# Orange-OpenSource/AIVC

Hardware: AMD Instinct MI355X
Metric: encode+decode fps @1080p YUV420 (RA GOP32) (higher is better)
Workload: dtype f32; 1 GPU; 1920x1080 8-bit YUV420, coding structure 1_GOP_32: one 128-frame clip = 4 intra-period units of 33 frames (132 coded frames, the last 4 repeat the last frame) encoded + decoded per step; synthetic random-init stand-in for model ms_ssim-4 (widths {'n2': 64, 'n': 128, 'c_y': 64, 'c_short': 64, 'c_z': 32, 'n_h': 128}), last analysis conv calibrated so that 6 (MOFNet) / 12 (CodecNet) of the 64 y featu; parallelism=single GPU

## Files before the change

### aivc_amd/csrc/conv_wino.hip

```cpp
#include <stdlib.h>

#include <type_traits>
#include <utility>

#include "common.h"

namespace aivc {

typedef float floatx16 __attribute__((ext_vector_type(16)));

struct WinoArgs {
  aivc_conv_params p;
  int TH, TW;
  int nby, nbx;
  int gy;
  int total;
  int poly;
  int cpp_shift;
};

__device__ __forceinline__ void wino_glds16(const float *base, uint32_t voff, uint32_t lds_dst) {
  asm volatile("s_mov_b32 m0, %2\n\ts_nop 0\n\tglobal_load_lds_dwordx4 %0, %1" : : "v"(voff), "s"(base), "s"(lds_dst) : "memory", "m0");
}

constexpr int WINO_RAW_STAGE = 11 * 1024;
constexpr int WINO_U_STAGE = 32 * 1024;
constexpr int WINO_V_QUAD = 1152;
constexpr int WINO_V_POS = 2 * WINO_V_QUAD;
constexpr int WINO_V_STAGE = 16 * WINO_V_POS;
constexpr int WINO_LDS = 2 * (WINO_RAW_STAGE + WINO_U_STAGE + WINO_V_STAGE);

__device__ __attribute__((aligned(4096))) float wino_zeros[1024];

template <int MODE>
__global__ __launch_bounds__(512) void conv_wino_kernel(WinoArgs a) {
  constexpr bool POLY = MODE == 1, TC = MODE == 2;
  extern __shared__ __attribute__((aligned(16))) char wsmem[];
  char *raw = wsmem, *Us = wsmem + 2 * WINO_RAW_STAGE, *Vs = Us + 2 * WINO_U_STAGE;
  const uint32_t lds0 = (uint32_t)(uintptr_t)(__attribute__((address_space(3))) char *)wsmem;

  const aivc_conv_params &p = a.p;
  const int tid = threadIdx.x, lane = tid & 63;
  const int wave = __builtin_amdgcn_readfirstlane(tid >> 6);
  const int ph = wave >> 2, wm = (wave >> 1) & 1, wn = wave & 1;
  const int H = TC ? p.h_in : p.h_out, W = TC ? p.w_in : p.w_out, Hi = p.h_in, Wi = p.w_in, Cin = p.c_in, Cout = p.c_out;
  const int gyc = TC ? 4 * a.gy : a.gy;
  constexpr int poly = POLY ? 1 : 0;
  const int cpp_shift = a.cpp_shift, cpp_mask = (1 << a.cpp_shift) - 1;

  const uint32_t total = (uint32_t)a.total, nwg = gridDim.x, xcd = blockIdx.x & 7u, slot = blockIdx.x >> 3;
  const uint32_t per_xcd = (total + 7u) >> 3, wg_per_xcd = (nwg + 7u - xcd) >> 3;
  const uint32_t x_lo = xcd * per_xcd, x_hi = min(x_lo + per_xcd, total);
  auto block_of = [&](uint32_t k) -> uint32_t { return x_lo + slot + k * wg_per_xcd; };
  const uint32_t n_mine = x_lo + slot < x_hi ? (x_hi - x_lo - slot + wg_per_xcd - 1u) / wg_per_xcd : 0u;
  if (n_mine == 0u) return;
  struct Desc {
    const float *xbase, *ubase;
    uint32_t r_off[2];
    int img, byi, bxi, cb;
  };
  int s_quad[2], s_py[2], s_px[2];
#pragma unroll
  for (int k = 0; k < 2; ++k) {
    int sl = 64 * (wave + 8 * k) + lane;
    sl = sl < 648 ? sl : 647;
    const int q2 = sl >> 1, plane = q2 / 81, rem = q2 - plane * 81, hy = rem / 9, hx = rem - hy * 9;
    s_quad[k] = sl & 1;
    s_py[k] = 2 * hy + (plane >> 1);
    s_px[k] = 2 * hx + (plane & 1);
  }
  const int nch = poly ? 4 * (Cin >> 3) : (Cin >> 3);
  auto make_desc = [&](uint32_t blk) {
    Desc d;
    d.cb = (int)(blk % (uint32_t)gyc);
    uint32_t rest = blk / (uint32_t)gyc;
    d.bxi = (int)(rest % (uint32_t)a.nbx);
    rest /= (uint32_t)a.nbx;
    d.byi = (int)(rest % (uint32_t)a.nby);
    d.img = (int)(rest / (uint32_t)a.nby);
    d.xbase = p.x + (size_t)d.img * (size_t)Hi * Wi * Cin;
    d.ubase = p.w_wino + (size_t)d.cb * (size_t)nch * (WINO_U_STAGE / 4);
    if constexpr (MODE == 0) {
#pragma unroll
      for (int k = 0; k < 2; ++k) {
        const int iy = max(min(16 * d.byi - 1 + s_py[k], Hi - 1), 0), ix = max(min(16 * d.bxi - 1 + s_px[k], Wi - 1), 0);
        d.r_off[k] = ((uint32_t)(iy * Wi + ix) * (uint32_t)Cin + (uint32_t)(4 * s_quad[k])) * 4u;
      }
    }
    return d;
  };
  uint32_t iss_off[2];
  auto patch_offsets = [&](const Desc &d_, int ph2) {
    const int st = poly ? 2 : 1, py = ph2 >> 1, px = ph2 & 1;
#pragma unroll
    for (int k = 0; k < 2; ++k) {
      const int iy = max(min(st * (16 * d_.byi - 1 + s_py[k]) + py, Hi - 1), 0), ix = max(min(st * (16 * d_.bxi - 1 + s_px[k]) + px, Wi - 1), 0);
      iss_off[k] = ((uint32_t)(iy * Wi + ix) * (uint32_t)Cin + (uint32_t)(4 * s_quad[k])) * 4u;
    }
  };
  uint64_t iss_addr[2];
  auto tc_addresses = [&](const Desc &d_) {
#pragma unroll
    for (int k = 0; k < 2; ++k) {
      const int iy = 16 * d_.byi - 1 + s_py[k], ix = 16 * d_.bxi - 1 + s_px[k];
      const bool in = iy >= 0 && iy < Hi && ix >= 0 && ix < Wi;
      const uint64_t a_in = (uint64_t)(uintptr_t)d_.xbase + ((uint64_t)((uint32_t)(iy * Wi + ix)) * (uint32_t)Cin + (uint32_t)(4 * s_quad[k])) * 4u;
      const uint64_t a_z = (uint64_t)(uintptr_t)wino_zeros + (uint32_t)(16 * s_quad[k]);
      iss_addr[k] = in ? a_in : a_z;
    }
  };
  Desc cur = make_desc(block_of(0)), nxt = n_mine > 1u ? make_desc(block_of(1)) : cur;

  const uint32_t r_dst = __builtin_amdgcn_readfirstlane(lds0 + (uint32_t)wave * 1024u);
  const uint32_t u_dst = __builtin_amdgcn_readfirstlane(lds0 + (uint32_t)(2 * WINO_RAW_STAGE) + (uint32_t)wave * 4096u);
  const uint32_t u_off = (uint32_t)(wave * 4096 + lane * 16);
  auto uniform_ptr = [](const float *q) -> const float * {
    const uint64_t v = (uint64_t)(uintptr_t)q;
    const uint32_t lo = __builtin_amdgcn_readfirstlane((uint32_t)v), hi = __builtin_amdgcn_readfirstlane((uint32_t)(v >> 32));
    return reinterpret_cast<const float *>((uintptr_t)(((uint64_t)hi << 32) | lo));
  };
  auto issue_raw = [&](const Desc &d_, int c) {
    const uint32_t d = r_dst + (uint32_t)((c & 1) * WINO_RAW_STAGE);
    if constexpr (TC) {
      if (c == 0) tc_addresses(d_);
      const uint32_t du = __builtin_amdgcn_readfirstlane(d);
      asm volatile("s_mov_b32 m0, %1\n\ts_nop 0\n\tglobal_load_lds_dwordx4 %0, off" : : "v"(iss_addr[0]), "s"(du) : "memory", "m0");
      if (wave < 3) asm volatile("s_mov_b32 m0, %1\n\ts_nop 0\n\tglobal_load_lds_dwordx4 %0, off" : : "v"(iss_addr[1]), "s"(du + 8192u) : "memory", "m0");
      iss_addr[0] += 32u;
      iss_addr[1] += 32u;
    } else if constexpr (POLY) {
      if ((c & cpp_mask) == 0) patch_offsets(d_, c >> cpp_shift);
      const float *src = uniform_ptr(d_.xbase + 8 * (c & cpp_mask));
      const uint32_t du = __builtin_amdgcn_readfirstlane(d);
      wino_glds16(src, iss_off[0], du);
      if (wave < 3) wino_glds16(src, iss_off[1], du + 8192u);
    } else {
      const float *src = d_.xbase + 8 * c;
      wino_glds16(src, d_.r_off[0], d);
      if (wave < 3) wino_glds16(src, d_.r_off[1], d + 8192u);
    }
  };
  auto zero_pos = [&](int pc, int i, int j) -> bool {
    if constexpr (POLY) return ((pc >> 1) && i == 3) || ((pc & 1) && j == 3);
    if constexpr (TC) return ((pc >> 1) && i == 0) || ((pc & 1) && j == 0);
    return false;
  };
  auto phase_or_class = [&](const Desc &d_, int c) -> int { return POLY ? c >> cpp_shift : (TC ? d_.cb / a.gy : 0); };
  auto issue_u = [&](const Desc &d_, int c) {
    const float *src = MODE != 0 ? uniform_ptr(d_.ubase + (size_t)c * (WINO_U_STAGE / 4)) : d_.ubase + (size_t)c * (WINO_U_STAGE / 4);
    const uint32_t d = MODE != 0 ? __builtin_amdgcn_readfirstlane(u_dst + (uint32_t)((c & 1) * WINO_U_STAGE)) : u_dst + (uint32_t)((c & 1) * WINO_U_STAGE);
    bool lo = true, hi = true;
    if constexpr (MODE != 0) {
      const int pc = phase_or_class(d_, c), i = wave >> 1, j = 2 * (wave & 1);
      lo = !zero_pos(pc, i, j);
      hi = !zero_pos(pc, i, j + 1);
    }
    if (lo && hi) {
      asm volatile("s_mov_b32 m0, %2\n\ts_nop 0\n\t"
                   "global_load_lds_dwordx4 %0, %1\n\t"
                   "global_load_lds_dwordx4 %0, %1 offset:1024\n\t"
                   "global_load_lds_dwordx4 %0, %1 offset:2048\n\t"
                   "global_load_lds_dwordx4 %0, %1 offset:3072"
                   : : "v"(u_off), "s"(src), "s"(d) : "memory", "m0");
    } else if (lo) {
      asm volatile("s_mov_b32 m0, %2\n\ts_nop 0\n\t"
                   "global_load_lds_dwordx4 %0, %1\n\t"
                   "global_load_lds_dwordx4 %0, %1 offset:1024"
                   : : "v"(u_off), "s"(src), "s"(d) : "memory", "m0");
    } else if (hi) {
      asm volatile("s_mov_b32 m0, %2\n\ts_nop 0\n\t"
                   "global_load_lds_dwordx4 %0, %1 offset:2048\n\t"
                   "global_load_lds_dwordx4 %0, %1 offset:3072"
                   : : "v"(u_off), "s"(src), "s"(d) : "memory", "m0");
    }
  };

  const int l32 = lane & 31;
  const int t_grp = (l32 < 4 || (l32 >= 12 && l32 < 16) || (l32 >= 20 && l32 < 28)) ? 0 : 1;
  const int t_pos = t_grp == 0 ? (l32 < 4 ? l32 : (l32 < 16 ? l32 - 8 : l32 - 12)) : (l32 < 12 ? l32 - 4 : (l32 < 20 ? l32 - 8 : l32 - 16));
  const int t_quad = t_pos >> 3, t_tx = (t_pos & 7) ^ (t_grp << 2), t_ty = ((tid >> 6) & 1) * 4 + (lane >> 5) * 2 + t_grp;
  const int t_i = __builtin_amdgcn_readfirstlane(tid >> 7);
  const int t_ra = t_i == 0 ? 0 : (t_i == 2 ? 2 : 1), t_rb = t_i == 3 ? 3 : (t_i == 2 ? 1 : 2);
  const float t_si = t_i == 1 ? 1.0f : -1.0f;
  const int t_base = ((t_ty * 9 + t_tx) * 2 + t_quad) * 16;
  auto pix_off = [](int r, int c) { return (((r & 1) * 2 + (c & 1)) * 81 + (r >> 1) * 9 + (c >> 1)) * 32; };
  int t_oa[4], t_ob[4];
#pragma unroll
  for (int c = 0; c < 4; ++c) {
    t_oa[c] = t_base + pix_off(t_ra, c);
    t_ob[c] = t_base + pix_off(t_rb, c);
  }
  const int t_vdst = (4 * t_i) * WINO_V_POS + t_quad * WINO_V_QUAD + (t_ty * 8 + t_tx) * 16;
  float4 R[4];
  auto comb = [](const float4 &u, const float4 &v, float sgn) {
    float4 o;
    o.x = __builtin_fmaf(sgn, v.x, u.x);
    o.y = __builtin_fmaf(sgn, v.y, u.y);
    o.z = __builtin_fmaf(sgn, v.z, u.z);
    o.w = __builtin_fmaf(sgn, v.w, u.w);
    return o;
  };
  auto transform_step = [&](auto STAGE, auto STEP) {
    constexpr int st = decltype(STEP)::value, stage = decltype(STAGE)::value;
    const char *rs = raw + stage * WINO_RAW_STAGE;
    char *vd = Vs + stage * WINO_V_STAGE + t_vdst;
    if constexpr (st < 4) {
      const float4 xa = *reinterpret_cast<const float4 *>(rs + t_oa[st]), xb = *reinterpret_cast<const float4 *>(rs + t_ob[st]);
      R[st] = comb(xa, xb, t_si);
    } else if constexpr (st == 4) {
      *reinterpret_cast<float4 *>(vd) = comb(R[0], R[2], -1.0f);
    } else if constexpr (st == 5) {
      *reinterpret_cast<float4 *>(vd + WINO_V_POS) = comb(R[1], R[2], 1.0f);
    } else if constexpr (st == 6) {
      *reinterpret_cast<float4 *>(vd + 2 * WINO_V_POS) = comb(R[2], R[1], -1.0f);
    } else {
      *reinterpret_cast<float4 *>(vd + 3 * WINO_V_POS) = comb(R[1], R[3], -1.0f);
    }
  };
  auto transform0 = [&]() {
    using std::integral_constant;
    using Z = integral_constant<int, 0>;
    transform_step(Z{}, integral_constant<int, 0>{});
    transform_step(Z{}, integral_constant<int, 1>{});
    transform_step(Z{}, integral_constant<int, 2>{});
    transform_step(Z{}, integral_constant<int, 3>{});
    transform_step(Z{}, integral_constant<int, 4>{});
    transform_step(Z{}, integral_constant<int, 5>{});
    transform_step(Z{}, integral_constant<int, 6>{});
    transform_step(Z{}, integral_constant<int, 7>{});
  };

  floatx16 acc[8];
#pragma unroll
  for (int q = 0; q < 8; ++q)
#pragma unroll
    for (int r = 0; r < 16; ++r) acc[q][r] = 0.0f;
  const int hh = lane >> 5, l31 = lane & 31;
  const int a_rd = (8 * ph) * WINO_V_POS + hh * WINO_V_QUAD + (32 * wm + l31) * 16;
  const int b_rd = (8 * ph) * 2048 + hh * 1024 + (32 * wn + l31) * 16;
  auto multiply = [&](auto STAGE, auto FIRST, uint32_t tm, uint32_t pm) {
    constexpr int stage = decltype(STAGE)::value;
    constexpr bool first = decltype(FIRST)::value;
    using NEXT = std::integral_constant<int, 1 - stage>;
    const char *va = Vs + stage * WINO_V_STAGE + a_rd, *ub = Us + stage * WINO_U_STAGE + b_rd;
    float4 af[2][2], bf[2][2];
    auto rd = [&](int set, int q) {
      af[set][0] = *reinterpret_cast<const float4 *>(va + q * WINO_V_POS);
      bf[set][0] = *reinterpret_cast<const float4 *>(ub + q * 2048);
      af[set][1] = *reinterpret_cast<const float4 *>(va + (q + 1) * WINO_V_POS);
      bf[set][1] = *reinterpret_cast<const float4 *>(ub + (q + 1) * 2048);
    };
    rd(0, 0);
    auto pair = [&](auto Q) {
      constexpr int q = decltype(Q)::value, set = (q >> 1) & 1;
      using std::integral_constant;
      if constexpr (q + 2 < 8) {
        if (MODE == 0 || (first && !TC) || (pm & (0xCu << q))) rd(1 - set, q + 2);
      }
      __builtin_amdgcn_sched_barrier(0);
      const float4 x0 = af[set][0], y0 = bf[set][0], x1 = af[set][1], y1 = bf[set][1];
#ifdef WINO_EXP_NOMFMA
      acc[q][0] += x0.x * y0.x + x0.y * y0.y + x0.z * y0.z + x0.w * y0.w;
      acc[q + 1][0] += x1.x * y1.x + x1.y * y1.y + x1.z * y1.z + x1.w * y1.w;
#else
      if constexpr (first && TC) {
        const floatx16 zero = {0.0f, 0.0f, 0.0f, 0.0f, 0.0f, 0.0f, 0.0f, 0.0f, 0.0f, 0.0f, 0.0f, 0.0f, 0.0f, 0.0f, 0.0f, 0.0f};
        if ((pm >> q) & 1u) {
          acc[q] = __builtin_amdgcn_mfma_f32_32x32x2f32(x0.x, y0.x, zero, 0, 0, 0);
          acc[q] = __builtin_amdgcn_mfma_f32_32x32x2f32(x0.y, y0.y, acc[q], 0, 0, 0);
          acc[q] = __builtin_amdgcn_mfma_f32_32x32x2f32(x0.z, y0.z, acc[q], 0, 0, 0);
          acc[q] = __builtin_amdgcn_mfma_f32_32x32x2f32(x0.w, y0.w, acc[q], 0, 0, 0);
        } else {
          acc[q] = __builtin_amdgcn_mfma_f32_32x32x2f32(0.0f, 0.0f, zero, 0, 0, 0);
        }
        if ((pm >> (q + 1)) & 1u) {
          acc[q + 1] = __builtin_amdgcn_mfma_f32_32x32x2f32(x1.x, y1.x, zero, 0, 0, 0);
          acc[q + 1] = __builtin_amdgcn_mfma_f32_32x32x2f32(x1.y, y1.y, acc[q + 1], 0, 0, 0);
          acc[q + 1] = __builtin_amdgcn_mfma_f32_32x32x2f32(x1.z, y1.z, acc[q + 1], 0, 0, 0);
          acc[q + 1] = __builtin_amdgcn_mfma_f32_32x32x2f32(x1.w, y1.w, acc[q + 1], 0, 0, 0);
        } else {
          acc[q + 1] = __builtin_amdgcn_mfma_f32_32x32x2f32(0.0f, 0.0f, zero, 0, 0, 0);
        }
      } else if constexpr (first) {
        const floatx16 zero = {0.0f, 0.0f, 0.0f, 0.0f, 0.0f, 0.0f, 0.0f, 0.0f, 0.0f, 0.0f, 0.0f, 0.0f, 0.0f, 0.0f, 0.0f, 0.0f};
        acc[q] = __builtin_amdgcn_mfma_f32_32x32x2f32(x0.x, y0.x, zero, 0, 0, 0);
        acc[q + 1] = __builtin_amdgcn_mfma_f32_32x32x2f32(x1.x, y1.x, zero, 0, 0, 0);
        acc[q] = __builtin_amdgcn_mfma_f32_32x32x2f32(x0.y, y0.y, acc[q], 0, 0, 0);
        acc[q + 1] = __builtin_amdgcn_mfma_f32_32x32x2f32(x1.y, y1.y, acc[q + 1], 0, 0, 0);
        acc[q] = __builtin_amdgcn_mfma_f32_32x32x2f32(x0.z, y0.z, acc[q], 0, 0, 0);
        acc[q + 1] = __builtin_amdgcn_mfma_f32_32x32x2f32(x1.z, y1.z, acc[q + 1], 0, 0, 0);
        acc[q] = __builtin_amdgcn_mfma_f32_32x32x2f32(x0.w, y0.w, acc[q], 0, 0, 0);
        acc[q + 1] = __builtin_amdgcn_mfma_f32_32x32x2f32(x1.w, y1.w, acc[q + 1], 0, 0, 0);
      } else {
        if (MODE == 0 || ((pm >> q) & 1u)) {
          acc[q] = __builtin_amdgcn_mfma_f32_32x32x2f32(x0.x, y0.x, acc[q], 0, 0, 0);
          acc[q] = __builtin_amdgcn_mfma_f32_32x32x2f32(x0.y, y0.y, acc[q], 0, 0, 0);
          acc[q] = __builtin_amdgcn_mfma_f32_32x32x2f32(x0.z, y0.z, acc[q], 0, 0, 0);
          acc[q] = __builtin_amdgcn_mfma_f32_32x32x2f32(x0.w, y0.w, acc[q], 0, 0, 0);
        }
        if (MODE == 0 || ((pm >> (q + 1)) & 1u)) {
          acc[q + 1] = __builtin_amdgcn_mfma_f32_32x32x2f32(x1.x, y1.x, acc[q + 1], 0, 0, 0);
          acc[q + 1] = __builtin_amdgcn_mfma_f32_32x32x2f32(x1.y, y1.y, acc[q + 1], 0, 0, 0);
          acc[q + 1] = __builtin_amdgcn_mfma_f32_32x32x2f32(x1.z, y1.z, acc[q + 1], 0, 0, 0);
          acc[q + 1] = __builtin_amdgcn_mfma_f32_32x32x2f32(x1.w, y1.w, acc[q + 1], 0, 0, 0);
        }
      }
#endif
      __builtin_amdgcn_sched_barrier(0);
#ifndef WINO_EXP_NOXFORM
      if ((tm >> q) & 1u) transform_step(NEXT{}, integral_constant<int, q>{});
      if ((tm >> (q + 1)) & 1u) transform_step(NEXT{}, integral_constant<int, q + 1>{});
#endif
      __builtin_amdgcn_sched_barrier(0);
    };
    using std::integral_constant;
    pair(integral_constant<int, 0>{});
    pair(integral_constant<int, 2>{});
    pair(integral_constant<int, 4>{});
    pair(integral_constant<int, 6>{});
  };

  auto issue_raw_at = [&](uint32_t kb, int c) {
    if (c < nch) issue_raw(cur, c);
    else if (kb + 1u < n_mine) issue_raw(nxt, c - nch);
  };
  auto issue_u_at = [&](uint32_t kb, int c) {
    if (c < nch) issue_u(cur, c);
    else if (kb + 1u < n_mine) issue_u(nxt, c - nch);
  };
  issue_raw(cur, 0);
  issue_u(cur, 0);
  issue_raw_at(0u, 1);
  asm volatile("s_waitcnt vmcnt(0)" ::: "memory");
  __builtin_amdgcn_s_barrier();
  transform0();
  asm volatile("s_waitcnt lgkmcnt(0)" ::: "memory");
  __builtin_amdgcn_s_barrier();
  const int act1 = p.act1, act2 = p.act2;
  auto act_cheap = [](int act, float v) {
    const float neg = act == AIVC_ACT_LEAKY ? v * 0.01f : (act == AIVC_ACT_RELU ? 0.0f : v);
    return v > 0.0f ? v : neg;
  };
  for (uint32_t kb = 0; kb < n_mine; ++kb) {
    auto chunk = [&](auto STAGE, auto FIRST, int c) {
#ifndef WINO_EXP_NODMA
      issue_raw_at(kb, c + 2);
      issue_u_at(kb, c + 1);
#endif
      uint32_t pm = 0xFFu;
      if (poly) {
        const int ph2 = c >> cpp_shift;
        pm = 0xFFu & ~((ph2 & 1) ? 0x88u : 0u) & ~(((ph2 >> 1) && ph) ? 0xF0u : 0u);
      }
      if constexpr (TC) {
        const int cls = cur.cb / a.gy;
        pm = 0xFFu & ~((cls & 1) ? 0x11u : 0u) & ~(((cls >> 1) && !ph) ? 0x0Fu : 0u);
      }
      uint32_t tm = (c + 1 < nch || kb + 1u < n_mine) ? 0xFFu : 0u;
      if constexpr (MODE != 0) {
        const int pcn = c + 1 < nch ? phase_or_class(cur, c + 1) : phase_or_class(nxt, 0);
        if (zero_pos(pcn, t_i, 1)) tm = 0u;
        else if (zero_pos(pcn, 1, POLY ? 3 : 0)) tm &= POLY ? ~0x80u : ~0x10u;
      }
      multiply(STAGE, FIRST, tm, pm);
      asm volatile("s_waitcnt vmcnt(0) lgkmcnt(0)" ::: "memory");
      __builtin_amdgcn_s_barrier();
    };
    {
      using std::integral_constant;
      using S0 = integral_constant<int, 0>;
      using S1 = integral_constant<int, 1>;
      chunk(S0{}, std::true_type{}, 0);
      chunk(S1{}, std::false_type{}, 1);
      for (int c = 2; c < nch; c += 2) {
        chunk(S0{}, std::false_type{}, c);
        chunk(S1{}, std::false_type{}, c + 1);
      }
    }

#ifdef WINO_EXP_NOEPI
    if (kb + 1u < n_mine) { cur = nxt; if (kb + 2u < n_mine) nxt = make_desc(block_of(kb + 2u)); continue; }
#endif
    floatx16 keep[2], give[2];
    auto fold = [&](auto PH) {
      constexpr int phc = decltype(PH)::value;
#pragma unroll
      for (int bb = 0; bb < 2; ++bb)
#pragma unroll
        for (int r = 0; r < 16; ++r) keep[bb][r] = give[bb][r] = 0.0f;
#pragma unroll
      for (int q = 0; q < 8; ++q) {
        const int i = 2 * phc + (q >> 2), j = q & 3;
        const int t0i = i < 3 ? 1 : 0, t1i = i == 0 ? 0 : (i == 1 ? 1 : -1);
        const int t0j = j < 3 ? 1 : 0, t1j = j == 0 ? 0 : (j == 1 ? 1 : -1);
#pragma unroll
        for (int o = 0; o < 4; ++o) {
          const int cf = ((o >> 1) ? t1i : t0i) * ((o & 1) ? t1j : t0j);
          floatx16 &dst = (o >> 1) == phc ? keep[o & 1] : give[o & 1];
          if (cf > 0) {
#pragma unroll
            for (int r = 0; r < 16; ++r) dst[r] = dst[r] + acc[q][r];
          } else if (cf < 0) {
#pragma unroll
            for (int r = 0; r < 16; ++r) dst[r] = dst[r] - acc[q][r];
          }
        }
      }
    };
    if (ph) fold(std::integral_constant<int, 1>{});
    else fold(std::integral_constant<int, 0>{});
    {
      float *xch = reinterpret_cast<float *>(Vs + WINO_V_STAGE) + wave * 1024;
      const float *theirs = reinterpret_cast<const float *>(Vs + WINO_V_STAGE) + (wave ^ 4) * 1024;
#pragma unroll
      for (int bb = 0; bb < 2; ++bb) {
#pragma unroll
        for (int r = 0; r < 16; ++r) xch[r * 64 + lane] = give[bb][r];
        asm volatile("s_waitcnt lgkmcnt(0)" ::: "memory");
        __builtin_amdgcn_s_barrier();
#pragma unroll
        for (int r = 0; r < 16; ++r) keep[bb][r] = keep[bb][r] + theirs[r * 64 + lane];
        asm volatile("s_waitcnt lgkmcnt(0)" ::: "memory");
        __builtin_amdgcn_s_barrier();
      }
    }

    {
      const float *__restrict__ g_mul = p.mul;
      const float *__restrict__ g_res = p.res;
      float *__restrict__ g_y = p.y;
      const int cls = TC ? cur.cb / a.gy : 0, pyc = cls >> 1, pxc = cls & 1;
      const int OS = TC ? 2 : 1;
      const int Wo_ = OS * W, Ho_ = OS * H;
      const int co = (TC ? cur.cb - cls * a.gy : cur.cb) * 64 + 32 * wn + l31;
      const bool has_bias = p.bias != nullptr;
      const float cbias = has_bias ? p.bias[co] : 0.0f;
      const int oy_w = 2 * (8 * cur.byi + 4 * wm) + ph;
      const bool inside_x = 16 * cur.bxi + 16 <= W;
      if (!g_mul && act1 != AIVC_ACT_SIGMOID) {
        const int cols_left = W - 16 * cur.bxi;
        typedef __attribute__((address_space(1))) char gchar;
        typedef __attribute__((address_space(1))) float gfloat;
        typedef __attribute__((address_space(1))) const float cgfloat;
        const uint32_t c4 = (uint32_t)Cout * 4u, sx = (uint32_t)OS * c4;
        uint32_t lane_b = (uint32_t)(2 * (8 * cur.bxi + 4 * hh)) * sx + (uint32_t)pxc * c4 + (uint32_t)co * 4u;
        asm volatile("" : "+v"(lane_b));
        const size_t img_b = (size_t)cur.img * (size_t)Ho_ * Wo_ * c4;
        auto rows = [&](auto RES, auto KIND, auto EDGE) {
          constexpr bool has_res = decltype(RES)::value;
          constexpr bool edge = decltype(EDGE)::value;
          constexpr int kind = decltype(KIND)::value;
          bool ok[8];
#pragma unroll
          for (int rr = 0; rr < 4; ++rr)
#pragma unroll
            for (int b = 0; b < 2; ++b) ok[rr * 2 + b] = !edge || 2 * (4 * hh + rr) + b < cols_left;
#pragma unroll
          for (int rq = 0; rq < 4; ++rq) {
            const int oy = oy_w + 2 * rq;
            if (oy >= H) continue;
            const size_t row_b = img_b + (size_t)(OS * oy + pyc) * Wo_ * c4;
            gchar *yb = (gchar *)(uintptr_t)(reinterpret_cast<char *>(g_y) + row_b);
            const gchar *rb = (const gchar *)(uintptr_t)(reinterpret_cast<const char *>(g_res) + row_b);
            float rv[8];
            if constexpr (has_res) {
#pragma unroll
              for (int rr = 0; rr < 4; ++rr)
#pragma unroll
                for (int b = 0; b < 2; ++b)
                  rv[rr * 2 + b] = ok[rr * 2 + b] ? *reinterpret_cast<cgfloat *>(rb + lane_b + (uint32_t)((2 * rr + b) * 512) * (sx / 512u)) : 0.0f;
            }
#pragma unroll
            for (int rr = 0; rr < 4; ++rr)
#pragma unroll
              for (int b = 0; b < 2; ++b) {
                const int r = rq * 4 + rr;
                float v = keep[b][r];
                if (has_bias) v = v + cbias;
                if constexpr (kind == 1) v = __builtin_fmaxf(v, v * 0.01f);
                if constexpr (kind == 2) v = v > 0.0f ? v : 0.0f;
                if constexpr (has_res) v = v + rv[rr * 2 + b];
                if constexpr (kind == 3) v = v > 0.0f ? v : 0.0f;
                if constexpr (kind == 4) v = __builtin_fmaxf(v, v * 0.01f);
#ifdef WINO_EXP_NOSTORE
                if (v == 123.456f)
#endif
                if (ok[rr * 2 + b]) *reinterpret_cast<gfloat *>(yb + lane_b + (uint32_t)((2 * rr + b) * 512) * (sx / 512u)) = v;
              }
          }
        };
        using std::integral_constant;
        int kind = -1;
        if (act1 == AIVC_ACT_NONE && act2 == AIVC_ACT_NONE) kind = 0;
        else if (act2 == AIVC_ACT_NONE) kind = act1 == AIVC_ACT_LEAKY ? 1 : 2;
        else if (act1 == AIVC_ACT_NONE) kind = act2 == AIVC_ACT_RELU ? 3 : 4;
        if (kind >= 0 && sx % 512u == 0u) {
          auto go = [&](auto RES, auto EDGE) {
            switch (kind) {
              case 0: rows(RES, integral_constant<int, 0>{}, EDGE); break;
              case 1: rows(RES, integral_constant<int, 1>{}, EDGE); break;
              case 2: rows(RES, integral_constant<int, 2>{}, EDGE); break;
              case 3: rows(RES, integral_constant<int, 3>{}, EDGE); break;
              default: rows(RES, integral_constant<int, 4>{}, EDGE); break;
            }
          };
          if (inside_x) {
            if (g_res) go(integral_constant<bool, true>{}, integral_constant<bool, false>{});
            else go(integral_constant<bool, false>{}, integral_constant<bool, false>{});
          } else {
            if (g_res) go(integral_constant<bool, true>{}, integral_constant<bool, true>{});
            else go(integral_constant<bool, false>{}, integral_constant<bool, true>{});
          }
          goto epilogue_done;
        }
      }
      {
        const size_t ybase = (size_t)cur.img * (size_t)Ho_ * Wo_ * Cout + (size_t)co;
#pragma unroll
        for (int r = 0; r < 16; ++r) {
          const int t = (r & 3) + 8 * (r >> 2) + 4 * hh;
          const int oy = oy_w + 2 * (t >> 3), ox0 = 2 * (8 * cur.bxi + (t & 7));
          if (oy >= H) continue;
#pragma unroll
          for (int b = 0; b < 2; ++b) {
            const int ox = ox0 + b;
            if (ox >= W) continue;
            const size_t o = ybase + ((size_t)(OS * oy + pyc) * Wo_ + (size_t)(OS * ox + pxc)) * (size_t)Cout;
            float v = keep[b][r];
            if (has_bias) v = v + cbias;
            v = act_cheap(act1, v);
            if (g_mul) v = g_mul[o] * v;
            if (g_res) v = v + g_res[o];
            v = act_cheap(act2, v);
#ifdef WINO_EXP_NOSTORE
            if (v == 123.456f)
#endif
            g_y[o] = v;
          }
        }
      }
    epilogue_done:;
    }
    cur = nxt;
    if (kb + 2u < n_mine) nxt = make_desc(block_of(kb + 2u));
  }
}

__device__ __forceinline__ void wino_g(double g0, double g1, double g2, double (&out)[4]) {
  out[0] = g0;
  out[1] = 0.5 * ((g0 + g1) + g2);
  out[2] = 0.5 * ((g0 - g1) + g2);
  out[3] = g2;
}
__global__ void __launch_bounds__(256) winograd_weights_kernel(const float *w, int c_out, int c_in, float *u) {
  const size_t idx = (size_t)blockIdx.x * 256 + threadIdx.x;
  if (idx >= (size_t)c_out * c_in) return;
  const int co = (int)(idx / c_in), ci = (int)(idx % c_in);
  double t[4][3], uu[4][4];
#pragma unroll
  for (int l = 0; l < 3; ++l) {
    double col[4];
    wino_g((double)w[(((size_t)co * 3 + 0) * 3 + l) * c_in + ci], (double)w[(((size_t)co * 3 + 1) * 3 + l) * c_in + ci],
           (double)w[(((size_t)co * 3 + 2) * 3 + l) * c_in + ci], col);
#pragma unroll
    for (int i = 0; i < 4; ++i) t[i][l] = col[i];
  }
#pragma unroll
  for (int i = 0; i < 4; ++i) wino_g(t[i][0], t[i][1], t[i][2], uu[i]);
#pragma unroll
  for (int i = 0; i < 4; ++i)
#pragma unroll
    for (int j = 0; j < 4; ++j) u[AIVC_WINO_U_INDEX(co, 4 * i + j, ci, c_in)] = (float)uu[i][j];
}

int winograd_weights(const float *w, int c_out, int c_in, float *u, hipStream_t s) {
  hipLaunchKernelGGL(winograd_weights_kernel, dim3(cdiv((size_t)c_out * c_in, 256)), dim3(256), 0, s, w, c_out, c_in, u);
  return check_launch("winograd_weights");
}

__global__ void __launch_bounds__(256) winograd_weights_poly5_kernel(const float *w, int c_out, int c_in, float *u) {
  const size_t idx = (size_t)blockIdx.x * 256 + threadIdx.x;
  if (idx >= (size_t)c_out * c_in * 4) return;
  const int phase = (int)(idx % 4), ci = (int)((idx / 4) % c_in), co = (int)(idx / ((size_t)4 * c_in));
  const int py = phase >> 1, px = phase & 1;
  auto tap = [&](int r, int l) -> double {
    const int ky = 2 * r + py, kx = 2 * l + px;
    return ky < 5 && kx < 5 ? (double)w[(((size_t)co * 5 + ky) * 5 + kx) * c_in + ci] : 0.0;
  };
  double t[4][3], uu[4][4];
#pragma unroll
  for (int l = 0; l < 3; ++l) {
    double col[4];
    wino_g(tap(0, l), tap(1, l), tap(2, l), col);
#pragma unroll
    for (int i = 0; i < 4; ++i) t[i][l] = col[i];
  }
#pragma unroll
  for (int i = 0; i < 4; ++i) wino_g(t[i][0], t[i][1], t[i][2], uu[i]);
#pragma unroll
  for (int i = 0; i < 4; ++i)
#pragma unroll
    for (int j = 0; j < 4; ++j) u[AIVC_WINO_U_INDEX(co, 4 * i + j, phase * c_in + ci, 4 * c_in)] = (float)uu[i][j];
}

int winograd_weights_poly5(const float *w, int c_out, int c_in, float *u, hipStream_t s) {
  hipLaunchKernelGGL(winograd_weights_poly5_kernel, dim3(cdiv((size_t)c_out * c_in * 4, 256)), dim3(256), 0, s, w, c_out, c_in, u);
  return check_launch("winograd_weights_poly5");
}

__global__ void __launch_bounds__(256) winograd_weights_tconv5_kernel(const float *w, int c_out, int c_in, float *u) {
  const size_t idx = (size_t)blockIdx.x * 256 + threadIdx.x;
  if (idx >= (size_t)c_out * c_in * 4) return;
  const int ci = (int)(idx % c_in), co = (int)((idx / c_in) % c_out), cls = (int)(idx / ((size_t)c_in * c_out));
  const int pyc = cls >> 1, pxc = cls & 1;
  auto tap = [&](int r, int l) -> double {
    const int ky = pyc + 4 - 2 * r, kx = pxc + 4 - 2 * l;
    return ky < 5 && kx < 5 ? (double)w[(((size_t)co * 5 + ky) * 5 + kx) * c_in + ci] : 0.0;
  };
  double t[4][3], uu[4][4];
#pragma unroll
  for (int l = 0; l < 3; ++l) {
    double col[4];
    wino_g(tap(0, l), tap(1, l), tap(2, l), col);
#pragma unroll
    for (int i = 0; i < 4; ++i) t[i][l] = col[i];
  }
#pragma unroll
  for (int i = 0; i < 4; ++i) wino_g(t[i][0], t[i][1], t[i][2], uu[i]);
#pragma unroll
  for (int i = 0; i < 4; ++i)
#pragma unroll
    for (int j = 0; j < 4; ++j) u[AIVC_WINO_U_INDEX(cls * c_out + co, 4 * i + j, ci, c_in)] = (float)uu[i][j];
}

int winograd_weights_tconv5(const float *w, int c_out, int c_in, float *u, hipStream_t s) {
  hipLaunchKernelGGL(winograd_weights_tconv5_kernel, dim3(cdiv((size_t)c_out * c_in * 4, 256)), dim3(256), 0, s, w, c_out, c_in, u);
  return check_launch("winograd_weights_tconv5");
}

bool conv2d_wino_supported(const aivc_conv_params &p) {
  if (!aivc_winograd_covers(&p) || p.gdn) return false;
  if ((uint64_t)p.h_in * p.w_in * p.c_in * 4u >= 0xFFFF0000ull) return false;
  const bool tc = p.mode == AIVC_MODE_TCONV;
  if (tc && p.c_in > 960) return false;
  const uint64_t gh = tc ? p.h_in : p.h_out, gw = tc ? p.w_in : p.w_out;
  const uint64_t blocks = (uint64_t)p.n * ((gh + 15) / 16) * ((gw + 15) / 16) * ((uint64_t)p.c_out / 64) * (tc ? 4 : 1);
  return blocks < 0x7FFFFFFFull;
}

int conv2d_wino_variant(const aivc_conv_params &p) { return p.mode == AIVC_MODE_TCONV ? 303 : (p.ksize == 5 ? 302 : 301); }

template <int MODE>
static int wino_launch(const WinoArgs &a, unsigned grid, hipStream_t s) {
  static LdsOptIn opt_in;
  if (!opt_in.raise(reinterpret_cast<const void *>(conv_wino_kernel<MODE>), WINO_LDS)) return check_launch("conv_wino lds attribute");
  hipLaunchKernelGGL(conv_wino_kernel<MODE>, dim3(grid), dim3(512), WINO_LDS, s, a);
  return check_launch("conv_wino");
}

int conv2d_wino(const aivc_conv_params &p, hipStream_t s) {
  if (!conv2d_wino_supported(p) || !p.w_wino) return AIVC_ERR_UNSUPPORTED;
  const bool tc = p.mode == AIVC_MODE_TCONV;
  WinoArgs a;
  a.p = p;
  a.poly = !tc && p.ksize == 5 ? 1 : 0;
  a.cpp_shift = 0;
  while ((8 << a.cpp_shift) < p.c_in) ++a.cpp_shift;
  a.TH = ((tc ? p.h_in : p.h_out) + 1) / 2;
  a.TW = ((tc ? p.w_in : p.w_out) + 1) / 2;
  a.nby = (a.TH + 7) / 8;
  a.nbx = (a.TW + 7) / 8;
  a.gy = p.c_out / 64;
  a.total = (int)((size_t)p.n * a.nby * a.nbx * a.gy * (tc ? 4 : 1));
  static std::atomic<int> n_cu{0};
  if (n_cu.load(std::memory_order_relaxed) == 0) {
    int dev = 0, cus = 0;
    n_cu = hipGetDevice(&dev) == hipSuccess && hipDeviceGetAttribute(&cus, hipDeviceAttributeMultiprocessorCount, dev) == hipSuccess && cus > 0 ? cus : 256;
  }
  unsigned grid = (unsigned)n_cu.load(std::memory_order_relaxed);
  if ((unsigned)a.total < grid) grid = (unsigned)a.total;
  if (tc) return wino_launch<2>(a, grid, s);
  return a.poly ? wino_launch<1>(a, grid, s) : wino_launch<0>(a, grid, s);
}

}
```

Baseline: 95.63 frames/s.

## Defer last MFMA pair of each Winograd chunk past next chunk's DMA issue

Moves the q=6 MFMA pair of each chunk into the start of the following chunk, where it runs after that chunk's raw/U global-to-LDS DMAs are issued. The aim is to issue the loads earlier and overlap the outstanding MFMAs with them, shortening the stall at the end-of-chunk waitcnt and barrier. The fragment registers are hoisted to kernel scope, so the previous chunk's operands stay live across the barrier; this raises register pressure and relies on the deferred pair still reading valid registers. The change also adds an optional LDS cycle-stamp probe, built only under WINO_STAMPS.

```diff
diff --git a/aivc_amd/csrc/conv_wino.hip b/aivc_amd/csrc/conv_wino.hip
--- a/aivc_amd/csrc/conv_wino.hip
+++ b/aivc_amd/csrc/conv_wino.hip
@@ -4,6 +4,10 @@
 #include <utility>
 
 #include "common.h"
+
+#ifndef WINO_DEFER_MASK
+#define WINO_DEFER_MASK 7
+#endif
 
 namespace aivc {
 
@@ -29,6 +33,15 @@
 constexpr int WINO_V_POS = 2 * WINO_V_QUAD;
 constexpr int WINO_V_STAGE = 16 * WINO_V_POS;
 constexpr int WINO_LDS = 2 * (WINO_RAW_STAGE + WINO_U_STAGE + WINO_V_STAGE);
+
+#ifdef WINO_STAMPS
+constexpr int WINO_STAMP_WGS = 32, WINO_STAMP_CHUNKS = 10, WINO_STAMP_FIRST = 2;
+constexpr int WINO_LDS_LAUNCH = WINO_LDS + 2048;
+static_assert(WINO_STAMP_CHUNKS * 8 * 6 * 4 <= 2048 && WINO_LDS_LAUNCH <= 160 * 1024, "stamps live in the LDS the stages leave");
+__device__ uint32_t wino_stamp_buf[WINO_STAMP_WGS * WINO_STAMP_CHUNKS * 8 * 6];
+#else
+constexpr int WINO_LDS_LAUNCH = WINO_LDS;
+#endif
 
 __device__ __attribute__((aligned(4096))) float wino_zeros[1024];
 
@@ -146,7 +159,7 @@
     return false;
   };
   auto phase_or_class = [&](const Desc &d_, int c) -> int { return POLY ? c >> cpp_shift : (TC ? d_.cb / a.gy : 0); };
-  auto issue_u = [&](const Desc &d_, int c) {
+  auto issue_u = [&](const Desc &d_, int c) -> int {
     const float *src = MODE != 0 ? uniform_ptr(d_.ubase + (size_t)c * (WINO_U_STAGE / 4)) : d_.ubase + (size_t)c * (WINO_U_STAGE / 4);
     const uint32_t d = MODE != 0 ? __builtin_amdgcn_readfirstlane(u_dst + (uint32_t)((c & 1) * WINO_U_STAGE)) : u_dst + (uint32_t)((c & 1) * WINO_U_STAGE);
     bool lo = true, hi = true;
@@ -173,6 +186,7 @@
                    "global_load_lds_dwordx4 %0, %1 offset:3072"
                    : : "v"(u_off), "s"(src), "s"(d) : "memory", "m0");
     }
+    return 2 * (int)lo + 2 * (int)hi;
   };
 
   const int l32 = lane & 31;
@@ -238,18 +252,85 @@
   const int hh = lane >> 5, l31 = lane & 31;
   const int a_rd = (8 * ph) * WINO_V_POS + hh * WINO_V_QUAD + (32 * wm + l31) * 16;
   const int b_rd = (8 * ph) * 2048 + hh * 1024 + (32 * wn + l31) * 16;
-  auto multiply = [&](auto STAGE, auto FIRST, uint32_t tm, uint32_t pm) {
-    constexpr int stage = decltype(STAGE)::value;
+  constexpr bool DEFER = ((WINO_DEFER_MASK) >> MODE) & 1;
+  float4 af[2][2], bf[2][2];
+  auto mfma_pair = [&](auto Q, auto FIRST, uint32_t pm) {
+    constexpr int q = decltype(Q)::value, set = (q >> 1) & 1;
+    constexpr bool first = decltype(FIRST)::value;
+    const float4 x0 = af[set][0], y0 = bf[set][0], x1 = af[set][1], y1 = bf[set][1];
+#ifdef WINO_EXP_NOMFMA
+    acc[q][0] += x0.x * y0.x + x0.y * y0.y + x0.z * y0.z + x0.w * y0.w;
+    acc[q + 1][0] += x1.x * y1.x + x1.y * y1.y + x1.z * y1.z + x1.w * y1.w;
+#else
+    if constexpr (first && TC) {
+      const floatx16 zero = {0.0f, 0.0f, 0.0f, 0.0f, 0.0f, 0.0f, 0.0f, 0.0f, 0.0f, 0.0f, 0.0f, 0.0f, 0.0f, 0.0f, 0.0f, 0.0f};
+      if ((pm >> q) & 1u) {
+        acc[q] = __builtin_amdgcn_mfma_f32_32x32x2f32(x0.x, y0.x, zero, 0, 0, 0);
+        acc[q] = __builtin_amdgcn_mfma_f32_32x32x2f32(x0.y, y0.y, acc[q], 0, 0, 0);
+        acc[q] = __builtin_amdgcn_mfma_f32_32x32x2f32(x0.z, y0.z, acc[q], 0, 0, 0);
+        acc[q] = __builtin_amdgcn_mfma_f32_32x32x2f32(x0.w, y0.w, acc[q], 0, 0, 0);
+      } else {
+        acc[q] = __builtin_amdgcn_mfma_f32_32x32x2f32(0.0f, 0.0f, zero, 0, 0, 0);
+      }
+      if ((pm >> (q + 1)) & 1u) {
+        acc[q + 1] = __builtin_amdgcn_mfma_f32_32x32x2f32(x1.x, y1.x, zero, 0, 0, 0);
+        acc[q + 1] = __builtin_amdgcn_mfma_f32_32x32x2f32(x1.y, y1.y, acc[q + 1], 0, 0, 0);
+        acc[q + 1] = __builtin_amdgcn_mfma_f32_32x32x2f32(x1.z, y1.z, acc[q + 1], 0, 0, 0);
+        acc[q + 1] = __builtin_amdgcn_mfma_f32_32x32x2f32(x1.w, y1.w, acc[q + 1], 0, 0, 0);
+      } else {
+        acc[q + 1] = __builtin_amdgcn_mfma_f32_32x32x2f32(0.0f, 0.0f, zero, 0, 0, 0);
+      }
+    } else if constexpr (first) {
+      const floatx16 zero = {0.0f, 0.0f, 0.0f, 0.0f, 0.0f, 0.0f, 0.0f, 0.0f, 0.0f, 0.0f, 0.0f, 0.0f, 0.0f, 0.0f, 0.0f, 0.0f};
+      acc[q] = __builtin_amdgcn_mfma_f32_32x32x2f32(x0.x, y0.x, zero, 0, 0, 0);
+      acc[q + 1] = __builtin_amdgcn_mfma_f32_32x32x2f32(x1.x, y1.x, zero, 0, 0, 0);
+      acc[q] = __builtin_amdgcn_mfma_f32_32x32x2f32(x0.y, y0.y, acc[q], 0, 0, 0);
+      acc[q + 1] = __builtin_amdgcn_mfma_f32_32x32x2f32(x1.y, y1.y, acc[q + 1], 0, 0, 0);
+      acc[q] = __builtin_amdgcn_mfma_f32_32x32x2f32(x0.z, y0.z, acc[q], 0, 0, 0);
+      acc[q + 1] = __builtin_amdgcn_mfma_f32_32x32x2f32(x1.z, y1.z, acc[q + 1], 0, 0, 0);
+      acc[q] = __builtin_amdgcn_mfma_f32_32x32x2f32(x0.w, y0.w, acc[q], 0, 0, 0);
+      acc[q + 1] = __builtin_amdgcn_mfma_f32_32x32x2f32(x1.w, y1.w, acc[q + 1], 0, 0, 0);
+    } else {
+      if (MODE == 0 || ((pm >> q) & 1u)) {
+        acc[q] = __builtin_amdgcn_mfma_f32_32x32x2f32(x0.x, y0.x, acc[q], 0, 0, 0);
+        acc[q] = __builtin_amdgcn_mfma_f32_32x32x2f32(x0.y, y0.y, acc[q], 0, 0, 0);
+        acc[q] = __builtin_amdgcn_mfma_f32_32x32x2f32(x0.z, y0.z, acc[q], 0, 0, 0);
+        acc[q] = __builtin_amdgcn_mfma_f32_32x32x2f32(x0.w, y0.w, acc[q], 0, 0, 0);
+      }
+      if (MODE == 0 || ((pm >> (q + 1)) & 1u)) {
+        acc[q + 1] = __builtin_amdgcn_mfma_f32_32x32x2f32(x1.x, y1.x, acc[q + 1], 0, 0, 0);
+        acc[q + 1] = __builtin_amdgcn_mfma_f32_32x32x2f32(x1.y, y1.y, acc[q + 1], 0, 0, 0);
+        acc[q + 1] = __builtin_amdgcn_mfma_f32_32x32x2f32(x1.z, y1.z, acc[q + 1], 0, 0, 0);
+        acc[q + 1] = __builtin_amdgcn_mfma_f32_32x32x2f32(x1.w, y1.w, acc[q + 1], 0, 0, 0);
+      }
+    }
+#endif
+  };
+  auto multiply = [&](auto STAGE, auto FIRST, auto DEF, uint32_t tm, uint32_t pm, uint32_t pmd, bool last, auto &&issue_dmas) {
+    constexpr int stage = decltype(STAGE)::value, def = decltype(DEF)::value;
     constexpr bool first = decltype(FIRST)::value;
     using NEXT = std::integral_constant<int, 1 - stage>;
     const char *va = Vs + stage * WINO_V_STAGE + a_rd, *ub = Us + stage * WINO_U_STAGE + b_rd;
-    float4 af[2][2], bf[2][2];
     auto rd = [&](int set, int q) {
       af[set][0] = *reinterpret_cast<const float4 *>(va + q * WINO_V_POS);
       bf[set][0] = *reinterpret_cast<const float4 *>(ub + q * 2048);
       af[set][1] = *reinterpret_cast<const float4 *>(va + (q + 1) * WINO_V_POS);
       bf[set][1] = *reinterpret_cast<const float4 *>(ub + (q + 1) * 2048);
     };
+    auto fresh = [&](int set) {
+#pragma unroll
+      for (int k = 0; k < 2; ++k) {
+        asm volatile("" : "=v"(af[set][k].x), "=v"(af[set][k].y), "=v"(af[set][k].z), "=v"(af[set][k].w));
+        asm volatile("" : "=v"(bf[set][k].x), "=v"(bf[set][k].y), "=v"(bf[set][k].z), "=v"(bf[set][k].w));
+      }
+    };
+    fresh(0);
+    if constexpr (!DEFER || def == 0) fresh(1);
+    if constexpr (DEFER && def != 0) {
+      mfma_pair(std::integral_constant<int, 6>{}, std::integral_constant<bool, def == 2>{}, pmd);
+      __builtin_amdgcn_sched_barrier(0);
+    }
+    issue_dmas();
     rd(0, 0);
     auto pair = [&](auto Q) {
       constexpr int q = decltype(Q)::value, set = (q >> 1) & 1;
@@ -258,54 +339,11 @@
         if (MODE == 0 || (first && !TC) || (pm & (0xCu << q))) rd(1 - set, q + 2);
       }
       __builtin_amdgcn_sched_barrier(0);
-      const float4 x0 = af[set][0], y0 = bf[set][0], x1 = af[set][1], y1 = bf[set][1];
-#ifdef WINO_EXP_NOMFMA
-      acc[q][0] += x0.x * y0.x + x0.y * y0.y + x0.z * y0.z + x0.w * y0.w;
-      acc[q + 1][0] += x1.x * y1.x + x1.y * y1.y + x1.z * y1.z + x1.w * y1.w;
-#else
-      if constexpr (first && TC) {
-        const floatx16 zero = {0.0f, 0.0f, 0.0f, 0.0f, 0.0f, 0.0f, 0.0f, 0.0f, 0.0f, 0.0f, 0.0f, 0.0f, 0.0f, 0.0f, 0.0f, 0.0f};
-        if ((pm >> q) & 1u) {
-          acc[q] = __builtin_amdgcn_mfma_f32_32x32x2f32(x0.x, y0.x, zero, 0, 0, 0);
-          acc[q] = __builtin_amdgcn_mfma_f32_32x32x2f32(x0.y, y0.y, acc[q], 0, 0, 0);
-          acc[q] = __builtin_amdgcn_mfma_f32_32x32x2f32(x0.z, y0.z, acc[q], 0, 0, 0);
-          acc[q] = __builtin_amdgcn_mfma_f32_32x32x2f32(x0.w, y0.w, acc[q], 0, 0, 0);
-        } else {
-          acc[q] = __builtin_amdgcn_mfma_f32_32x32x2f32(0.0f, 0.0f, zero, 0, 0, 0);
-        }
-        if ((pm >> (q + 1)) & 1u) {
-          acc[q + 1] = __builtin_amdgcn_mfma_f32_32x32x2f32(x1.x, y1.x, zero, 0, 0, 0);
-          acc[q + 1] = __builtin_amdgcn_mfma_f32_32x32x2f32(x1.y, y1.y, acc[q + 1], 0, 0, 0);
-          acc[q + 1] = __builtin_amdgcn_mfma_f32_32x32x2f32(x1.z, y1.z, acc[q + 1], 0, 0, 0);
-          acc[q + 1] = __builtin_amdgcn_mfma_f32_32x32x2f32(x1.w, y1.w, acc[q + 1], 0, 0, 0);
-        } else {
-          acc[q + 1] = __builtin_amdgcn_mfma_f32_32x32x2f32(0.0f, 0.0f, zero, 0, 0, 0);
-        }
-      } else if constexpr (first) {
-        const floatx16 zero = {0.0f, 0.0f, 0.0f, 0.0f, 0.0f, 0.0f, 0.0f, 0.0f, 0.0f, 0.0f, 0.0f, 0.0f, 0.0f, 0.0f, 0.0f, 0.0f};
-        acc[q] = __builtin_amdgcn_mfma_f32_32x32x2f32(x0.x, y0.x, zero, 0, 0, 0);
-        acc[q + 1] = __builtin_amdgcn_mfma_f32_32x32x2f32(x1.x, y1.x, zero, 0, 0, 0);
-        acc[q] = __builtin_amdgcn_mfma_f32_32x32x2f32(x0.y, y0.y, acc[q], 0, 0, 0);
-        acc[q + 1] = __builtin_amdgcn_mfma_f32_32x32x2f32(x1.y, y1.y, acc[q + 1], 0, 0, 0);
-        acc[q] = __builtin_amdgcn_mfma_f32_32x32x2f32(x0.z, y0.z, acc[q], 0, 0, 0);
-        acc[q + 1] = __builtin_amdgcn_mfma_f32_32x32x2f32(x1.z, y1.z, acc[q + 1], 0, 0, 0);
-        acc[q] = __builtin_amdgcn_mfma_f32_32x32x2f32(x0.w, y0.w, acc[q], 0, 0, 0);
-        acc[q + 1] = __builtin_amdgcn_mfma_f32_32x32x2f32(x1.w, y1.w, acc[q + 1], 0, 0, 0);
+      if constexpr (DEFER && q == 6) {
+        if (last) mfma_pair(Q, FIRST, pm);
       } else {
-        if (MODE == 0 || ((pm >> q) & 1u)) {
-          acc[q] = __builtin_amdgcn_mfma_f32_32x32x2f32(x0.x, y0.x, acc[q], 0, 0, 0);
-          acc[q] = __builtin_amdgcn_mfma_f32_32x32x2f32(x0.y, y0.y, acc[q], 0, 0, 0);
-          acc[q] = __builtin_amdgcn_mfma_f32_32x32x2f32(x0.z, y0.z, acc[q], 0, 0, 0);
-          acc[q] = __builtin_amdgcn_mfma_f32_32x32x2f32(x0.w, y0.w, acc[q], 0, 0, 0);
-        }
-        if (MODE == 0 || ((pm >> (q + 1)) & 1u)) {
-          acc[q + 1] = __builtin_amdgcn_mfma_f32_32x32x2f32(x1.x, y1.x, acc[q + 1], 0, 0, 0);
-          acc[q + 1] = __builtin_amdgcn_mfma_f32_32x32x2f32(x1.y, y1.y, acc[q + 1], 0, 0, 0);
-          acc[q + 1] = __builtin_amdgcn_mfma_f32_32x32x2f32(x1.z, y1.z, acc[q + 1], 0, 0, 0);
-          acc[q + 1] = __builtin_amdgcn_mfma_f32_32x32x2f32(x1.w, y1.w, acc[q + 1], 0, 0, 0);
-        }
-      }
-#endif
+        mfma_pair(Q, FIRST, pm);
+      }
       __builtin_amdgcn_sched_barrier(0);
 #ifndef WINO_EXP_NOXFORM
       if ((tm >> q) & 1u) transform_step(NEXT{}, integral_constant<int, q>{});
@@ -324,9 +362,10 @@
     if (c < nch) issue_raw(cur, c);
     else if (kb + 1u < n_mine) issue_raw(nxt, c - nch);
   };
-  auto issue_u_at = [&](uint32_t kb, int c) {
-    if (c < nch) issue_u(cur, c);
-    else if (kb + 1u < n_mine) issue_u(nxt, c - nch);
+  auto issue_u_at = [&](uint32_t kb, int c) -> int {
+    if (c < nch) return issue_u(cur, c);
+    if (kb + 1u < n_mine) return issue_u(nxt, c - nch);
+    return 0;
   };
   issue_raw(cur, 0);
   issue_u(cur, 0);
@@ -341,12 +380,31 @@
     const float neg = act == AIVC_ACT_LEAKY ? v * 0.01f : (act == AIVC_ACT_RELU ? 0.0f : v);
     return v > 0.0f ? v : neg;
   };
+  uint32_t pm_prev = 0xFFu;
   for (uint32_t kb = 0; kb < n_mine; ++kb) {
-    auto chunk = [&](auto STAGE, auto FIRST, int c) {
+    auto chunk = [&](auto STAGE, auto FIRST, auto DEF, int c) {
+#ifdef WINO_STAMPS
+      const bool st_on = kb == 1u && c >= WINO_STAMP_FIRST && c < WINO_STAMP_FIRST + WINO_STAMP_CHUNKS;
+      uint32_t *st_row = reinterpret_cast<uint32_t *>(wsmem + WINO_LDS) + ((c - WINO_STAMP_FIRST) * 8 + wave) * 6;
+#define WINO_STAMP(i)                                                   \
+  if (st_on) {                                                          \
+    const uint32_t st_t = (uint32_t)__builtin_readcyclecounter();       \
+    if (lane == 0) st_row[i] = st_t;                                    \
+  }
+      WINO_STAMP(0)
+#endif
+      int u_cnt = 0;
+      auto issue_dmas = [&]() {
 #ifndef WINO_EXP_NODMA
-      issue_raw_at(kb, c + 2);
-      issue_u_at(kb, c + 1);
-#endif
+        issue_raw_at(kb, c + 2);
+        u_cnt = issue_u_at(kb, c + 1);
+#endif
+#ifdef WINO_STAMPS
+        WINO_STAMP(1)
+#else
+        (void)u_cnt;
+#endif
+      };
       uint32_t pm = 0xFFu;
       if (poly) {
         const int ph2 = c >> cpp_shift;
@@ -362,20 +420,46 @@
         if (zero_pos(pcn, t_i, 1)) tm = 0u;
         else if (zero_pos(pcn, 1, POLY ? 3 : 0)) tm &= POLY ? ~0x80u : ~0x10u;
       }
-      multiply(STAGE, FIRST, tm, pm);
+      multiply(STAGE, FIRST, DEF, tm, pm, pm_prev, decltype(STAGE)::value == 1 && c + 1 == nch, issue_dmas);
+      pm_prev = TC ? 0xFFu : pm;
+#ifdef WINO_STAMPS
+      asm volatile("s_waitcnt lgkmcnt(0)" ::: "memory");
+      WINO_STAMP(2)
+      if (u_cnt == 4) asm volatile("s_waitcnt vmcnt(4)" ::: "memory");
+      else if (u_cnt == 2) asm volatile("s_waitcnt vmcnt(2)" ::: "memory");
+      else asm volatile("s_waitcnt vmcnt(0)" ::: "memory");
+      WINO_STAMP(3)
+      asm volatile("s_waitcnt vmcnt(0)" ::: "memory");
+      WINO_STAMP(4)
+      asm volatile("s_waitcnt lgkmcnt(0)" ::: "memory");
+      __builtin_amdgcn_s_barrier();
+      WINO_STAMP(5)
+#undef WINO_STAMP
+#else
       asm volatile("s_waitcnt vmcnt(0) lgkmcnt(0)" ::: "memory");
       __builtin_amdgcn_s_barrier();
+#endif
     };
     {
       using std::integral_constant;
       using S0 = integral_constant<int, 0>;
       using S1 = integral_constant<int, 1>;
-      chunk(S0{}, std::true_type{}, 0);
-      chunk(S1{}, std::false_type{}, 1);
+      using D0 = integral_constant<int, 0>;
+      using D1 = integral_constant<int, 1>;
+      using D2 = integral_constant<int, 2>;
+      chunk(S0{}, std::true_type{}, D0{}, 0);
+      chunk(S1{}, std::false_type{}, D2{}, 1);
       for (int c = 2; c < nch; c += 2) {
-        chunk(S0{}, std::false_type{}, c);
-        chunk(S1{}, std::false_type{}, c + 1);
-      }
+        chunk(S0{}, std::false_type{}, D1{}, c);
+        chunk(S1{}, std::false_type{}, D1{}, c + 1);
+      }
+#ifdef WINO_STAMPS
+      if (kb == 1u && blockIdx.x < WINO_STAMP_WGS && nch >= WINO_STAMP_FIRST + WINO_STAMP_CHUNKS && lane < WINO_STAMP_CHUNKS * 6) {
+        const int sc = lane / 6, si = lane - 6 * sc;
+        wino_stamp_buf[((blockIdx.x * WINO_STAMP_CHUNKS + sc) * 8 + wave) * 6 + si] =
+            reinterpret_cast<const uint32_t *>(wsmem + WINO_LDS)[(sc * 8 + wave) * 6 + si];
+      }
+#endif
     }
 
 #ifdef WINO_EXP_NOEPI
@@ -653,8 +737,8 @@
 template <int MODE>
 static int wino_launch(const WinoArgs &a, unsigned grid, hipStream_t s) {
   static LdsOptIn opt_in;
-  if (!opt_in.raise(reinterpret_cast<const void *>(conv_wino_kernel<MODE>), WINO_LDS)) return check_launch("conv_wino lds attribute");
-  hipLaunchKernelGGL(conv_wino_kernel<MODE>, dim3(grid), dim3(512), WINO_LDS, s, a);
+  if (!opt_in.raise(reinterpret_cast<const void *>(conv_wino_kernel<MODE>), WINO_LDS_LAUNCH)) return check_launch("conv_wino lds attribute");
+  hipLaunchKernelGGL(conv_wino_kernel<MODE>, dim3(grid), dim3(512), WINO_LDS_LAUNCH, s, a);
   return check_launch("conv_wino");
 }
 
@@ -683,4 +767,13 @@
   return a.poly ? wino_launch<1>(a, grid, s) : wino_launch<0>(a, grid, s);
 }
 
-}
+#ifdef WINO_STAMPS
+extern "C" __attribute__((visibility("default"))) int aivc_dbg_wino_stamps(uint32_t *out, int n) {
+  constexpr int total = WINO_STAMP_WGS * WINO_STAMP_CHUNKS * 8 * 6;
+  if (hipDeviceSynchronize() != hipSuccess) return -1;
+  if (hipMemcpyFromSymbol(out, HIP_SYMBOL(wino_stamp_buf), sizeof(uint32_t) * (size_t)(n < total ? n : total)) != hipSuccess) return -1;
+  return n < total ? n : total;
+}
+#endif
+
+}
```

New measurement: 95.49 frames/s. No clear change (-0.1%).
